# darglein/Snake-SLAM

Measured on AMD Instinct MI355X. Metric: frames/s ORB extract+match @752x480, higher is better.
Workload: dtype u8

## Files before the change

### snake_slam_amd/csrc/dispatch.hpp

```cpp
#pragma once
#include <cstddef>

#ifndef SNK_POSE_RED_STEPS
#define SNK_POSE_RED_STEPS 2
#endif

namespace snk
{
constexpr int BF_MFMA_MIN      = 24;
constexpr int BF_WIDE_MIN_WORK = 16384;

enum class Knn2Form { vector1, vector4, mfma };

inline Knn2Form knn2_form(int nq_cap, int nt_cap, int batch, bool no_mfma)
{
    if (!no_mfma && nq_cap >= BF_MFMA_MIN && nt_cap >= BF_MFMA_MIN) return Knn2Form::mfma;
    return (long long)batch * nq_cap >= BF_WIDE_MIN_WORK ? Knn2Form::vector4 : Knn2Form::vector1;
}

constexpr int BF_MFMA_WIDE_MIN_WGS = 512;

constexpr bool knn2_mfma_wide(int nq_cap, int , int batch, int wide_env)
{
    return wide_env >= 0 ? wide_env != 0 : (long long)batch * ((nq_cap + 255) / 256) >= BF_MFMA_WIDE_MIN_WGS;
}

constexpr int BF_MFMA_SHORT_NT = 8192;

constexpr bool knn2_mfma_short(int nt_cap, bool allowed) { return allowed && nt_cap <= BF_MFMA_SHORT_NT; }

constexpr int ST_SORT_MAX     = 8192;
constexpr int ST_FRAME_MAX    = 2560;
constexpr int ST_FRAME_BATCH  = 8;
constexpr int ST_COUNT_ROWS   = 4096;

enum class StereoForm { frame, count16, sort16, unindexed };

inline StereoForm stereo_host_form(int nr, bool sort_network)
{
    if (nr > ST_SORT_MAX) return StereoForm::unindexed;
    return sort_network ? StereoForm::sort16 : StereoForm::count16;
}

inline StereoForm stereo_batch_form(int nr_cap, int batch, bool no_frame_kernel, bool sort_network)
{
    if (!no_frame_kernel && nr_cap <= ST_FRAME_MAX && batch >= ST_FRAME_BATCH) return StereoForm::frame;
    return stereo_host_form(nr_cap, sort_network);
}

constexpr int POSE_SLOTS_PER_WAVE   = 64 >> SNK_POSE_RED_STEPS;
constexpr int POSE_HOST_WAVE4_MEAN  = 192;
constexpr int POSE_BATCH_WAVE4_MIN  = 256;
constexpr int POSE_TWO_PER_CU_BATCH = 256;
constexpr int POSE_MATCH_BYTES      = 56;

enum class PoseForm { wave1, wave2_lds, wave4_lds, wave4_global };

constexpr int pose_dyn_max() { return 160 * 1024 - (4 * POSE_SLOTS_PER_WAVE * 28 + 28) * 8 - 2048; }
constexpr int pose_two_per_cu() { return (80 * 1024 - (4 * POSE_SLOTS_PER_WAVE * 28 + 28) * 8 - 256) / POSE_MATCH_BYTES; }
constexpr int pose_four_per_cu() { return (160 * 1024 / 4 - (2 * POSE_SLOTS_PER_WAVE * 28 + 28) * 8 - 512) / POSE_MATCH_BYTES; }

inline PoseForm pose_host_form(size_t total, int n_problems, bool no_lds)
{
    if (total < (size_t)n_problems * POSE_HOST_WAVE4_MEAN) return PoseForm::wave1;
    return no_lds ? PoseForm::wave4_global : PoseForm::wave4_lds;
}

inline int pose_host_carve(int n_max, int n_problems)
{
    int lds_matches = n_max;
    if (n_problems > POSE_TWO_PER_CU_BATCH && lds_matches > pose_two_per_cu()) lds_matches = pose_two_per_cu();
    if ((size_t)lds_matches * POSE_MATCH_BYTES > (size_t)pose_dyn_max()) lds_matches = pose_dyn_max() / POSE_MATCH_BYTES;
    return lds_matches;
}

inline bool pose_batch_two_waves(int batch, int n_cu, int waves_env) { return waves_env == 2 || (waves_env != 4 && batch > 2 * n_cu); }

inline PoseForm pose_batch_form(int stride, int batch, int n_cu, int waves_env, bool no_lds)
{
    if (stride < POSE_BATCH_WAVE4_MIN) return PoseForm::wave1;
    if (no_lds) return PoseForm::wave4_global;
    return pose_batch_two_waves(batch, n_cu, waves_env) ? PoseForm::wave2_lds : PoseForm::wave4_lds;
}

inline int pose_batch_carve(int stride, int batch, int lds_env, bool two_waves)
{
    int lds_matches = stride;
    if (two_waves)
    {
        const int lm = lds_env > 0 ? lds_env : pose_four_per_cu();
        lds_matches  = lm < stride ? lm : stride;
    }
    else if (lds_env > 0) lds_matches = lds_env < stride ? lds_env : stride;
    else if (batch > POSE_TWO_PER_CU_BATCH && lds_matches > pose_two_per_cu()) lds_matches = pose_two_per_cu();
    if ((size_t)lds_matches * POSE_MATCH_BYTES > (size_t)pose_dyn_max()) lds_matches = pose_dyn_max() / POSE_MATCH_BYTES;
    return lds_matches;
}
}
```

### snake_slam_amd/csrc/matcher.hip

```cpp
#include "common.hpp"
#include "dispatch.hpp"

namespace snk
{
namespace
{
using u32 = unsigned int;
using u64 = unsigned long long;

constexpr u32 BF_IDX_BITS = 20;
constexpr u32 BF_IDX_MASK = (1u << BF_IDX_BITS) - 1u;
constexpr u32 BF_INF_KEY  = ((u32)SNK_DIST_INF << BF_IDX_BITS) | BF_IDX_MASK;

__device__ __forceinline__ int hamming256(const uint4& a0, const uint4& a1, const uint4& b0, const uint4& b1)
{
    return __popc(a0.x ^ b0.x) + __popc(a0.y ^ b0.y) + __popc(a0.z ^ b0.z) + __popc(a0.w ^ b0.w) +
           __popc(a1.x ^ b1.x) + __popc(a1.y ^ b1.y) + __popc(a1.z ^ b1.z) + __popc(a1.w ^ b1.w);
}

template <typename K>
__device__ __forceinline__ void merge2(K& k1, K& k2, K o1, K o2)
{
    K lo = k1 < o1 ? k1 : o1;
    K hi = k1 < o1 ? o1 : k1;
    K m  = k2 < o2 ? k2 : o2;
    k2   = hi < m ? hi : m;
    k1   = lo;
}

template <typename K>
__device__ __forceinline__ void insert2(K& k1, K& k2, K key)
{
    K hi = k1 < key ? key : k1;
    k1   = k1 < key ? k1 : key;
    k2   = k2 < hi ? k2 : hi;
}

template <int QW>
__global__ __launch_bounds__(256) void bf_knn2_kernel(const uint4* __restrict__ query, const int* __restrict__ nq_dev,
                                                      int nq_cap, int nq_host, const uint4* __restrict__ train,
                                                      const int* __restrict__ nt_dev, int nt_cap, int nt_host,
                                                      snk_knn2* __restrict__ out)
{
    const int b    = blockIdx.y;
    int nq         = nq_dev ? nq_dev[b] : nq_host;
    int nt         = nt_dev ? nt_dev[b] : nt_host;
    nq             = nq < nq_cap ? nq : nq_cap;
    nt             = nt < nt_cap ? nt : nt_cap;
    const int wave = __builtin_amdgcn_readfirstlane(threadIdx.x >> 6);
    const int lane = threadIdx.x & 63;
    const int q0   = (blockIdx.x * 4 + wave) * QW;
    if (q0 >= nq) return;

    const uint4* qb = query + (size_t)b * nq_cap * 2;
    const uint4* tb = train + (size_t)b * nt_cap * 2;

    uint4 qa[QW], qc[QW];
    u32 k1[QW], k2[QW];
#pragma unroll
    for (int k = 0; k < QW; ++k)
    {
        int qi = q0 + k < nq ? q0 + k : nq - 1;
        qa[k]  = qb[(size_t)qi * 2];
        qc[k]  = qb[(size_t)qi * 2 + 1];
        k1[k]  = BF_INF_KEY;
        k2[k]  = BF_INF_KEY;
    }

    for (int j = lane; j < nt; j += 64)
    {
        const uint4 ta = tb[(size_t)j * 2];
        const uint4 tc = tb[(size_t)j * 2 + 1];
#pragma unroll
        for (int k = 0; k < QW; ++k)
        {
            u32 d   = (u32)hamming256(qa[k], qc[k], ta, tc);
            u32 key = d < (u32)SNK_DIST_INF ? ((d << BF_IDX_BITS) | (u32)j) : BF_INF_KEY;
            insert2(k1[k], k2[k], key);
        }
    }

#pragma unroll
    for (int off = 32; off >= 1; off >>= 1)
    {
#pragma unroll
        for (int k = 0; k < QW; ++k)
        {
            u32 o1 = __shfl_xor(k1[k], off);
            u32 o2 = __shfl_xor(k2[k], off);
            merge2(k1[k], k2[k], o1, o2);
        }
    }

    if (lane == 0)
    {
#pragma unroll
        for (int k = 0; k < QW; ++k)
        {
            if (q0 + k < nq)
            {
                snk_knn2 r;
                r.dist1 = (int)(k1[k] >> BF_IDX_BITS);
                r.idx1  = (k1[k] & BF_IDX_MASK) == BF_IDX_MASK ? -1 : (int)(k1[k] & BF_IDX_MASK);
                r.dist2 = (int)(k2[k] >> BF_IDX_BITS);
                r.idx2  = (k2[k] & BF_IDX_MASK) == BF_IDX_MASK ? -1 : (int)(k2[k] & BF_IDX_MASK);
                out[(size_t)b * nq_cap + q0 + k] = r;
            }
        }
    }
}

typedef int v4i __attribute__((ext_vector_type(4)));
typedef int v16i __attribute__((ext_vector_type(16)));
constexpr int BFM_SENTINEL = 0x7F000000;
constexpr u32 BFS_IDX_BITS = 13;
static_assert(BF_MFMA_SHORT_NT == 1 << BFS_IDX_BITS, "the SHORT key's index field holds every index below BF_MFMA_SHORT_NT");

template <bool SHORT>
__device__ __forceinline__ v4i expand_bits(const uint4& h, int kc)
{
    if constexpr (SHORT)
    {
        const u32 M = 0x80808080u;
        return v4i{(int)((h.x << (7 - kc)) & M), (int)((h.y << (7 - kc)) & M), (int)((h.z << (7 - kc)) & M), (int)((h.w << (7 - kc)) & M)};
    }
    const u32 M = 0x01010101u;
    return v4i{(int)((h.x >> kc) & M), (int)((h.y >> kc) & M), (int)((h.z >> kc) & M), (int)((h.w >> kc) & M)};
}
__device__ __forceinline__ int popc128(const uint4& h) { return __popc(h.x) + __popc(h.y) + __popc(h.z) + __popc(h.w); }
__device__ __forceinline__ int med3s(int a, int b, int c) { return max(min(a, b), min(max(a, b), c)); }
template <bool MAXK>
__device__ __forceinline__ void insert2s(int& k1, int& k2, int key)
{
    k2 = med3s(k1, k2, key);
    k1 = MAXK ? max(k1, key) : min(k1, key);
}

template <int NB, bool SHORT>
__global__ __launch_bounds__(256, 2) void bf_knn2_mfma_kernel(const uint4* __restrict__ query, const int* __restrict__ nq_dev,
                                                              int nq_cap, int nq_host, const uint4* __restrict__ train,
                                                              const int* __restrict__ nt_dev, int nt_cap, int nt_host,
                                                              snk_knn2* __restrict__ out)
{
    __shared__ v4i As[2][8 * 2 * 32];
    __shared__ v16i ptk[2][2];
    constexpr int NONE = SHORT ? -BFM_SENTINEL : BFM_SENTINEL;
    const int b = blockIdx.y;
    int nq      = nq_dev ? nq_dev[b] : nq_host;
    int nt      = nt_dev ? nt_dev[b] : nt_host;
    nq          = nq < nq_cap ? nq : nq_cap;
    nt          = nt < nt_cap ? nt : nt_cap;
    if ((int)blockIdx.x * (128 * NB) >= nq) return;
    const int wave = __builtin_amdgcn_readfirstlane(threadIdx.x >> 6), lane = threadIdx.x & 63;
    const int j = lane & 31, g = lane >> 5;
    const int q0 = (blockIdx.x * 4 + wave) * (32 * NB);
    const uint4* qb = query + (size_t)b * nq_cap * 2;
    const uint4* tb = train + (size_t)b * nt_cap * 2;

    int pq[NB];
    v4i B[NB][8];
#pragma unroll
    for (int n = 0; n < NB; ++n)
    {
        const int qi   = min(q0 + 32 * n + j, nq - 1);
        const uint4 qh = qb[(size_t)qi * 2 + g], qo = qb[(size_t)qi * 2 + (1 - g)];
        pq[n]          = popc128(qh) + popc128(qo);
#pragma unroll
        for (int kc = 0; kc < 8; ++kc) {
            const v4i e = expand_bits<SHORT>(qh, kc);
            if constexpr (SHORT) B[n][kc] = e;
            else B[n][kc] = v4i{(int)((u32)e.x * 0xFFu), (int)((u32)e.y * 0xFFu), (int)((u32)e.z * 0xFFu), (int)((u32)e.w * 0xFFu)};
        }
    }

    const int e_i = wave * 8 + (lane & 7), e_g = (lane >> 3) & 1, e_k = lane >> 4;
    const int e_p = ((e_i >> 2) & 1) * 16 + (e_i & 3) + 4 * (e_i >> 3);
    const int ntiles = (nt + 31) >> 5;
    auto fetch = [&](int t, uint4& h)
    {
        const int ti = t * 32 + e_i;
        h = uint4{0u, 0u, 0u, 0u};
        if (ti < nt) h = tb[(size_t)ti * 2 + e_g];
    };
    auto expand = [&](int t, int buf, const uint4& h)
    {
        As[buf][((2 * e_k) * 2 + e_g) * 32 + e_i]     = expand_bits<SHORT>(h, 2 * e_k);
        As[buf][((2 * e_k + 1) * 2 + e_g) * 32 + e_i] = expand_bits<SHORT>(h, 2 * e_k + 1);
        const int ph = popc128(h);
        const int pt = ph + __shfl_down(ph, 8);
        if (lane < 8)
        {
            const int ti = t * 32 + e_i;
            const int k  = SHORT ? -((pt << BFS_IDX_BITS) | ti) : ((pt << BF_IDX_BITS) | ti);
            reinterpret_cast<int*>(&ptk[buf][0])[e_p] = ti < nt ? k : NONE;
        }
    };

    int k1[NB], k2[NB];
#pragma unroll
    for (int n = 0; n < NB; ++n) k1[n] = k2[n] = NONE;
    uint4 h;
    if (ntiles > 0)
    {
        fetch(0, h);
        expand(0, 0, h);
        if (ntiles > 1) fetch(1, h);
    }
    __syncthreads();
    for (int t = 0; t < ntiles; ++t)
    {
        const int buf = t & 1;
        if (t + 1 < ntiles)
        {
            expand(t + 1, buf ^ 1, h);
            if (t + 2 < ntiles) fetch(t + 2, h);
        }
        v16i acc[NB];
        v4i a[8];
#pragma unroll
        for (int kc = 0; kc < 8; ++kc) a[kc] = As[buf][(kc * 2 + g) * 32 + j];
        const v16i pk = ptk[buf][g];
#pragma unroll
        for (int n = 0; n < NB; ++n)
        {
            acc[n] = SHORT ? pk : v16i{0, 0, 0, 0, 0, 0, 0, 0, 0, 0, 0, 0, 0, 0, 0, 0};
#pragma unroll
            for (int kc = 0; kc < 8; ++kc) acc[n] = __builtin_amdgcn_mfma_i32_32x32x32_i8(a[kc], B[n][kc], acc[n], 0, 0, 0);
        }
#pragma unroll
        for (int n = 0; n < NB; ++n)
#pragma unroll
            for (int r = 0; r < 16; ++r)
            {
                if constexpr (SHORT) insert2s<true>(k1[n], k2[n], acc[n][r]);
                else insert2s<false>(k1[n], k2[n], (int)(((u32)acc[n][r] << (BF_IDX_BITS + 1)) + (u32)pk[r]));
            }
        __builtin_amdgcn_sched_group_barrier(0x100, SHORT ? 12 : 8, 0);
        __builtin_amdgcn_sched_group_barrier(0x008, 8, 0);
        if constexpr (!SHORT) __builtin_amdgcn_sched_group_barrier(0x100, 4, 0);
        __syncthreads();
    }
#pragma unroll
    for (int n = 0; n < NB; ++n)
    {
        const int o1 = __shfl_xor(k1[n], 32), o2 = __shfl_xor(k2[n], 32);
        int r1, r2;
        if constexpr (SHORT) r1 = -max(k1[n], o1), r2 = -max(min(k1[n], o1), max(k2[n], o2));
        else r1 = min(k1[n], o1), r2 = min(max(k1[n], o1), min(k2[n], o2));
        if (lane < 32 && q0 + 32 * n + lane < nq)
        {
            constexpr u32 IB = SHORT ? BFS_IDX_BITS : BF_IDX_BITS, IM = (1u << IB) - 1u;
            snk_knn2 r;
            const int a1 = r1 >= BFM_SENTINEL - (1 << 30) ? -1 : r1 + (pq[n] << IB);
            const int a2 = r2 >= BFM_SENTINEL - (1 << 30) ? -1 : r2 + (pq[n] << IB);
            const bool v1 = a1 >= 0 && (a1 >> IB) < SNK_DIST_INF, v2 = a2 >= 0 && (a2 >> IB) < SNK_DIST_INF;
            r.dist1 = v1 ? a1 >> IB : SNK_DIST_INF;
            r.idx1  = v1 ? (int)((u32)a1 & IM) : -1;
            r.dist2 = v2 ? a2 >> IB : SNK_DIST_INF;
            r.idx2  = v2 ? (int)((u32)a2 & IM) : -1;
            out[(size_t)b * nq_cap + q0 + 32 * n + lane] = r;
        }
    }
}

__global__ __launch_bounds__(256) void bf_filter_kernel(const snk_knn2* __restrict__ knn, const int* __restrict__ nq_dev,
                                                        int nq_cap, int nq_host, int threshold, float ratio, int th_strict,
                                                        int ratio_strict, int2* __restrict__ pairs, int* __restrict__ n_pairs)
{
    __shared__ int wave_cnt[4];
    __shared__ int base_s;
    const int b    = blockIdx.x;
    int nq         = nq_dev ? nq_dev[b] : nq_host;
    nq             = nq < nq_cap ? nq : nq_cap;
    const int tid  = threadIdx.x;
    const int wave = tid >> 6;
    const int lane = tid & 63;
    if (tid == 0) base_s = 0;
    __syncthreads();
    for (int start = 0; start < nq; start += 256)
    {
        const int i = start + tid;
        bool keep   = false;
        snk_knn2 k  = {};
        if (i < nq)
        {
            k    = knn[(size_t)b * nq_cap + i];
            const float rd2 = ratio * (float)k.dist2;
            keep = k.idx1 >= 0 && (th_strict ? k.dist1 < threshold : k.dist1 <= threshold) &&
                   (ratio_strict ? (float)k.dist1 < rd2 : (float)k.dist1 <= rd2);
        }
        const u64 mask   = __ballot(keep);
        const int prefix = __popcll(mask & ((1ull << lane) - 1ull));
        if (lane == 0) wave_cnt[wave] = __popcll(mask);
        __syncthreads();
        int off = base_s;
        for (int w = 0; w < wave; ++w) off += wave_cnt[w];
        if (keep) pairs[(size_t)b * nq_cap + off + prefix] = make_int2(i, k.idx1);
        __syncthreads();
        if (tid == 0) base_s += wave_cnt[0] + wave_cnt[1] + wave_cnt[2] + wave_cnt[3];
        __syncthreads();
    }
    if (tid == 0) n_pairs[b] = base_s;
}

struct LevelScales
{
    float s[32];
    int n;
    int iround_mode;
};

__device__ __forceinline__ int iround_d(double x, int mode)
{
    if (mode == 0) return (int)floor(x + 0.5);
    if (mode == 1) return (int)(x < 0.0 ? -floor(0.5 - x) : floor(x + 0.5));
    return (int)rint(x);
}

constexpr u64 ST_INF_KEY = (250ull << 40) | 0xFFFFFFFFFFull;
constexpr int ST_ROW_BIAS    = 4096;

__device__ __forceinline__ void stereo_sort_network(const snk_kp64* __restrict__ rb, int nr, int iround_mode, u32* keys, u32* __restrict__ out)
{
    const int tid = threadIdx.x;
    int n_pow2    = 2;
    while (n_pow2 < nr) n_pow2 <<= 1;
    for (int i = tid; i < n_pow2; i += 256)
    {
        u32 k = 0xFFFFFFFFu;
        if (i < nr)
        {
            int row = iround_d(rb[i].y, iround_mode) + ST_ROW_BIAS;
            row     = row < 0 ? 0 : (row > 65535 ? 65535 : row);
            k       = ((u32)row << 16) | (u32)i;
        }
        keys[i] = k;
    }
    __syncthreads();
    for (int k = 2; k <= n_pow2; k <<= 1)
        for (int j = k >> 1; j > 0; j >>= 1)
        {
            for (int t = tid; t < (n_pow2 >> 1); t += 256)
            {
                const int i   = ((t & ~(j - 1)) << 1) | (t & (j - 1));
                const int ixj = i | j;
                const bool up = (i & k) == 0;
                const u32 x = keys[i], y = keys[ixj];
                if ((x > y) == up)
                {
                    keys[i]   = y;
                    keys[ixj] = x;
                }
            }
            __syncthreads();
        }
    for (int i = tid; i < nr; i += 256) out[i] = keys[i];
}
__global__ __launch_bounds__(256) void stereo_sort_kernel(const snk_kp64* __restrict__ right, const int* __restrict__ nr_dev,
                                                          int nr_cap, int nr_host, int iround_mode, u32* __restrict__ row_sorted)
{
    extern __shared__ __attribute__((aligned(16))) unsigned char ssm[];
    const int b = blockIdx.x;
    int nr      = nr_dev ? nr_dev[b] : nr_host;
    nr          = nr < nr_cap ? nr : nr_cap;
    stereo_sort_network(right + (size_t)b * nr_cap, nr, iround_mode, reinterpret_cast<u32*>(ssm), row_sorted + (size_t)b * nr_cap);
}

__global__ __launch_bounds__(256) void stereo_count_kernel(const snk_kp64* __restrict__ right, const int* __restrict__ nr_dev, int nr_cap,
                                                           int nr_host, int iround_mode, u32* __restrict__ row_sorted,
                                                           int* __restrict__ n_matches, float* __restrict__ prefill_rp,
                                                           float* __restrict__ prefill_dp, int prefill_n)
{
    extern __shared__ __attribute__((aligned(16))) unsigned char ssm[];
    if (n_matches && threadIdx.x == 0) n_matches[blockIdx.x] = 0;
    if (prefill_rp)
        for (int i = threadIdx.x; i < prefill_n; i += 256)
        {
            prefill_rp[(size_t)blockIdx.x * prefill_n + i] = -1000.0f;
            prefill_dp[(size_t)blockIdx.x * prefill_n + i] = -1000.0f;
        }
    __shared__ int s_min, s_max, s_wsum[4];
    int* start   = reinterpret_cast<int*>(ssm);
    int* fill    = start + ST_COUNT_ROWS + 1;
    int* rowof   = fill + ST_COUNT_ROWS + 1;
    int* seg     = rowof + nr_cap;
    const int b = blockIdx.x, tid = threadIdx.x, lane = tid & 63, wave = tid >> 6;
    int nr      = nr_dev ? nr_dev[b] : nr_host;
    nr          = nr < nr_cap ? nr : nr_cap;
    const snk_kp64* rb = right + (size_t)b * nr_cap;
    if (tid == 0) s_min = 65535, s_max = 0;
    __syncthreads();
    int lmin = 65535, lmax = 0;
    for (int i = tid; i < nr; i += 256)
    {
        int row = iround_d(rb[i].y, iround_mode) + ST_ROW_BIAS;
        row     = row < 0 ? 0 : (row > 65535 ? 65535 : row);
        rowof[i] = row;
        lmin = min(lmin, row), lmax = max(lmax, row);
    }
    atomicMin(&s_min, lmin);
    atomicMax(&s_max, lmax);
    __syncthreads();
    const int r0 = s_min, span = nr > 0 ? s_max - s_min + 1 : 1;
    if (span > ST_COUNT_ROWS)
// ... 323 lines not shown
            row[u]  = min(row[u] - row0, ST_ROWS - 1);
            rank[u] = atomicAdd(&start[row[u]], 1);
        }
    __syncthreads();
    {
        const int a = start[2 * tid], c = start[2 * tid + 1];
        int x       = a + c;
        x = wave_scan_incl_dpp(x);
        if ((tid & 63) == 63) s_wtot[tid >> 6] = x;
        __syncthreads();
        int base = 0;
        for (int w = 0; w < (tid >> 6); ++w) base += s_wtot[w];
        const int excl     = base + x - (a + c);
        start[2 * tid]     = excl;
        start[2 * tid + 1] = excl + a;
        if (tid == 1023) start[ST_ROWS] = base + x;
    }
    __syncthreads();
#pragma unroll
    for (int u = 0; u < PER; ++u)
        if (row[u] >= 0) srt[start[row[u]] + rank[u]] = tid + 1024 * u;
    __syncthreads();

    constexpr int NGRP = 1024 / ST_GROUP;
    const int lane = tid % ST_GROUP, grp = tid / ST_GROUP;
    const float max_disp = (float)(bf * 0.5);
    snk_kp64 kp_n = lb[min(grp, nl - 1)];
    uint4 qa_n = dlb[(size_t)min(grp, nl - 1) * 2], qc_n = dlb[(size_t)min(grp, nl - 1) * 2 + 1];
    for (int i = grp; i < nl; i += NGRP)
    {
        const snk_kp64 kp = kp_n;
        const uint4 qa = qa_n, qc = qc_n;
        {
            const int in = min(i + NGRP, nl - 1);
            kp_n = lb[in];
            qa_n = dlb[(size_t)in * 2];
            qc_n = dlb[(size_t)in * 2 + 1];
        }
        const int y = iround_d(kp.y, ls.iround_mode);
        int oct     = kp.octave;
        oct         = oct < 0 ? 0 : (oct >= ls.n ? ls.n - 1 : oct);
        const int ri = (int)ceilf(2.0f * ls.s[oct]);
        const int lo_row  = min(max(y - ri + ST_ROW_BIAS, 0), 65535), hi_row = min(max(y + ri + ST_ROW_BIAS, 0), 65535);
        const int scan_lo = start[min(max(lo_row - row0, 0), ST_ROWS - 1)], scan_hi = start[min(max(hi_row - row0, 0), ST_ROWS - 1) + 1];
        u64 k1 = ST_INF_KEY, k2 = ST_INF_KEY;
        for (int pos = scan_lo + lane; pos < scan_hi; pos += ST_GROUP)
        {
            const int j   = srt[pos];
            const int rel = syj[j] - (y - ri);
            if (rel < 0 || rel > 2 * ri) continue;
            const double disparity = kp.x - sx[j];
            if (disparity < 0.0 || disparity > (double)max_disp) continue;
            int doct = kp.octave - soct[j];
            doct     = doct < 0 ? -doct : doct;
            if (doct > 1) continue;
            const int dist = hamming256(qa, qc, sdesc[2 * j], sdesc[2 * j + 1]);
            if (dist >= 250) continue;
            insert2(k1, k2, ((u64)dist << 40) | ((u64)rel << 24) | (u64)j);
        }
#pragma unroll
        for (int off = ST_GROUP / 2; off >= 1; off >>= 1)
        {
            const u64 o1 = __shfl_xor(k1, off, 16), o2 = __shfl_xor(k2, off, 16);
            merge2(k1, k2, o1, o2);
        }
        if (lane != 0) continue;
        const int best_dist = (int)(k1 >> 40), second_best_dist = (int)(k2 >> 40);
        if (best_dist > (relaxed ? 75 : 40)) continue;
        if ((double)best_dist > (relaxed ? 0.9 : 0.7) * (double)second_best_dist) continue;
        const int best_id  = (int)(k1 & 0xFFFFFFull);
        const float angle1 = kp.angle, angle2 = sang[best_id];
        const float rot    = fminf(fabsf(angle1 - angle2), fminf(fabsf((angle1 + 365.0f) - angle2), fabsf(angle1 - (angle2 + 365.0f))));
        if (rot > (relaxed ? 25.0f : 5.0f)) continue;
        double right_point = sx[best_id];
        double disparity   = kp.x - right_point;
        if (disparity <= 0.001)
        {
            disparity   = 0.001;
            right_point = kp.x - disparity;
        }
        right_points[(size_t)b * nl_cap + i] = (float)right_point;
        depth[(size_t)b * nl_cap + i]        = (float)(bf / disparity);
        atomicAdd(&s_cnt, 1);
    }
    __syncthreads();
    if (tid == 0) n_matches[b] = s_cnt;
}
}
}

using namespace snk;

#include "matcher_handle.hpp"

extern "C" {

int snk_matcher_destroy(snk_matcher* m);

int snk_matcher_create(int device, void* stream, snk_matcher** out)
{
    SNK_REQUIRE(out != nullptr, "out is NULL");
    *out           = nullptr;
    snk_matcher* m = new snk_matcher();
    int rc         = m->init(device, stream);
    constexpr size_t SCRATCH = 4u << 20;
    for (snk::DevBuf* b : {&m->q, &m->t, &m->out, &m->aux, &m->aux2, &m->view})
        if (rc == SNK_OK) rc = b->reserve(SCRATCH);
    if (rc == SNK_OK) rc = m->cnt.reserve(256);
    if (rc == SNK_OK) rc = m->h_in.reserve(1u << 20);
    if (rc == SNK_OK) rc = m->h_res.reserve(256u << 10);
    if (rc != SNK_OK)
    {
        snk_matcher_destroy(m);
        return rc;
    }
    *out = m;
    return SNK_OK;
}

int snk_matcher_destroy(snk_matcher* m)
{
    if (!m) return SNK_OK;
    (void)hipSetDevice(m->device);
    m->q.release();
    m->t.release();
    m->out.release();
    m->aux.release();
    m->aux2.release();
    m->cnt.release();
    m->view.release();
    m->h_in.release();
    m->h_res.release();
    m->sim3_its.release();
    m->sim3_its_host.release();
    m->fini();
    delete m;
    return SNK_OK;
}

int snk_matcher_sync(snk_matcher* m)
{
    SNK_REQUIRE(m != nullptr, "matcher is NULL");
    SNK_HIP_CHECK(hipStreamSynchronize(m->stream));
    return SNK_OK;
}

static int launch_knn2(snk_matcher* m, const uint64_t* q, const int32_t* nq_dev, int nq_cap, int nq_host,
                       const uint64_t* t, const int32_t* nt_dev, int nt_cap, int nt_host, int batch, snk_knn2* out)
{
    if (batch <= 0 || nq_cap <= 0) return SNK_OK;
    static const bool no_mfma = getenv("SNK_BF_NO_MFMA") != nullptr;
    static const int wide_env  = getenv("SNK_BF_MFMA_WIDE") ? (atoi(getenv("SNK_BF_MFMA_WIDE")) != 0 ? 1 : 0) : -1;
    static const bool short_env = getenv("SNK_BF_MFMA_NO_SHORT") == nullptr;
    switch (knn2_form(nq_cap, nt_cap, batch, no_mfma))
    {
    case Knn2Form::mfma:
    {
        const bool wide = knn2_mfma_wide(nq_cap, nt_cap, batch, wide_env), shrt = knn2_mfma_short(nt_cap, short_env);
        auto kernel = wide ? (shrt ? bf_knn2_mfma_kernel<2, true> : bf_knn2_mfma_kernel<2, false>)
                           : (shrt ? bf_knn2_mfma_kernel<1, true> : bf_knn2_mfma_kernel<1, false>);
        hipLaunchKernelGGL(kernel, dim3(ceil_div(nq_cap, wide ? 256 : 128), batch), dim3(256), 0, m->stream, (const uint4*)q, nq_dev, nq_cap,
                           nq_host, (const uint4*)t, nt_dev, nt_cap, nt_host, out);
    }
        break;
    case Knn2Form::vector4:
        hipLaunchKernelGGL(bf_knn2_kernel<4>, dim3(ceil_div(nq_cap, 16), batch), dim3(256), 0, m->stream, (const uint4*)q, nq_dev, nq_cap,
                           nq_host, (const uint4*)t, nt_dev, nt_cap, nt_host, out);
        break;
    case Knn2Form::vector1:
        hipLaunchKernelGGL(bf_knn2_kernel<1>, dim3(ceil_div(nq_cap, 4), batch), dim3(256), 0, m->stream, (const uint4*)q, nq_dev, nq_cap,
                           nq_host, (const uint4*)t, nt_dev, nt_cap, nt_host, out);
        break;
    }
    SNK_LAUNCH_CHECK();
    return SNK_OK;
}

int snk_bf_knn2(snk_matcher* m, const uint64_t (*query)[4], int nq, const uint64_t (*train)[4], int nt, snk_knn2* out)
{
    SNK_REQUIRE(m != nullptr, "matcher is NULL");
    SNK_REQUIRE(nq >= 0 && nt >= 0, "negative count");
    SNK_REQUIRE(nt < (int)BF_IDX_MASK, "train set too large (max 2^20-2)");
    if (nq == 0) return SNK_OK;
    SNK_REQUIRE(query != nullptr && out != nullptr, "NULL buffer");
    SNK_REQUIRE(nt == 0 || train != nullptr, "NULL train buffer");
    SNK_HIP_CHECK(hipSetDevice(m->device));
    int rc;
    const size_t qb = (size_t)nq * 32, tb = (size_t)(nt > 0 ? nt : 1) * 32, ob = (size_t)nq * sizeof(snk_knn2);
    if ((rc = m->q.reserve(qb + tb)) != SNK_OK) return rc;
    if ((rc = m->out.reserve(ob)) != SNK_OK) return rc;
    if ((rc = m->h_in.reserve(qb + tb)) != SNK_OK) return rc;
    if ((rc = m->h_res.reserve(ob)) != SNK_OK) return rc;
    memcpy(m->h_in.p, query, qb);
    if (nt > 0) memcpy(m->h_in.as<char>() + qb, train, (size_t)nt * 32);
    SNK_HIP_CHECK(hipMemcpyAsync(m->q.p, m->h_in.p, qb + (nt > 0 ? (size_t)nt * 32 : 0), hipMemcpyHostToDevice, m->stream));
    rc = launch_knn2(m, m->q.as<uint64_t>(), nullptr, nq, nq, reinterpret_cast<const uint64_t*>(m->q.as<char>() + qb), nullptr,
                     nt > 0 ? nt : 1, nt, 1, m->out.as<snk_knn2>());
    if (rc != SNK_OK) return rc;
    SNK_HIP_CHECK(hipMemcpyAsync(m->h_res.p, m->out.p, ob, hipMemcpyDeviceToHost, m->stream));
    SNK_HIP_CHECK(hipStreamSynchronize(m->stream));
    memcpy(out, m->h_res.p, ob);
    return SNK_OK;
}

int snk_bf_knn2_batch_dev(snk_matcher* m, const uint64_t* query_dev, const int32_t* nq_dev, int nq_cap,
                          const uint64_t* train_dev, const int32_t* nt_dev, int nt_cap, int batch, snk_knn2* out_dev)
{
    SNK_REQUIRE(m != nullptr, "matcher is NULL");
    SNK_REQUIRE(batch >= 0 && nq_cap >= 0 && nt_cap >= 1, "bad sizes");
    SNK_REQUIRE(nt_cap < (int)BF_IDX_MASK, "train capacity too large (max 2^20-2)");
    SNK_REQUIRE(query_dev && train_dev && out_dev && nq_dev && nt_dev, "NULL device buffer");
    SNK_HIP_CHECK(hipSetDevice(m->device));
    return launch_knn2(m, query_dev, nq_dev, nq_cap, 0, train_dev, nt_dev, nt_cap, 0, batch, out_dev);
}

int snk_bf_filter(snk_matcher* m, const snk_knn2* knn, int nq, int threshold, float ratio, int32_t (*pairs)[2],
                  int* n_pairs)
{
    SNK_REQUIRE(m != nullptr, "matcher is NULL");
    SNK_REQUIRE(nq >= 0, "negative count");
    SNK_REQUIRE(n_pairs != nullptr, "n_pairs is NULL");
    *n_pairs = 0;
    if (nq == 0) return SNK_OK;
    SNK_REQUIRE(knn != nullptr && pairs != nullptr, "NULL buffer");
    SNK_HIP_CHECK(hipSetDevice(m->device));
    int rc;
    const size_t kb = (size_t)nq * sizeof(snk_knn2), pb = 16 + (size_t)nq * 8;
    if ((rc = m->out.reserve(kb)) != SNK_OK) return rc;
    if ((rc = m->aux.reserve(pb)) != SNK_OK) return rc;
    if ((rc = m->h_in.reserve(kb)) != SNK_OK) return rc;
    if ((rc = m->h_res.reserve(pb)) != SNK_OK) return rc;
    memcpy(m->h_in.p, knn, kb);
    SNK_HIP_CHECK(hipMemcpyAsync(m->out.p, m->h_in.p, kb, hipMemcpyHostToDevice, m->stream));
    hipLaunchKernelGGL(bf_filter_kernel, dim3(1), dim3(256), 0, m->stream, m->out.as<snk_knn2>(), (const int*)nullptr,
                       nq, nq, threshold, ratio, definition(DEF_BF_FILTER_THRESHOLD_STRICT), definition(DEF_BF_FILTER_RATIO_STRICT),
                       reinterpret_cast<int2*>(m->aux.as<char>() + 16), m->aux.as<int>());
    SNK_LAUNCH_CHECK();
    SNK_HIP_CHECK(hipMemcpyAsync(m->h_res.p, m->aux.p, pb, hipMemcpyDeviceToHost, m->stream));
    SNK_HIP_CHECK(hipStreamSynchronize(m->stream));
    const int n = *m->h_res.as<int>();
    if (n > 0) memcpy(pairs, m->h_res.as<char>() + 16, (size_t)n * 8);
    *n_pairs = n;
    return SNK_OK;
}

int snk_bf_filter_batch_dev(snk_matcher* m, const snk_knn2* knn_dev, const int32_t* nq_dev, int nq_cap, int batch,
                            int threshold, float ratio, int32_t* pairs_dev, int32_t* n_pairs_dev)
{
    SNK_REQUIRE(m != nullptr, "matcher is NULL");
    SNK_REQUIRE(batch >= 0 && nq_cap >= 0, "bad sizes");
    SNK_REQUIRE(knn_dev && nq_dev && pairs_dev && n_pairs_dev, "NULL device buffer");
    if (batch == 0) return SNK_OK;
    SNK_HIP_CHECK(hipSetDevice(m->device));
    hipLaunchKernelGGL(bf_filter_kernel, dim3(batch), dim3(256), 0, m->stream, knn_dev, nq_dev, nq_cap, 0, threshold,
                       ratio, definition(DEF_BF_FILTER_THRESHOLD_STRICT), definition(DEF_BF_FILTER_RATIO_STRICT), (int2*)pairs_dev,
                       n_pairs_dev);
    SNK_LAUNCH_CHECK();
    return SNK_OK;
}

static int make_scales(const float* level_scale, int n_levels, LevelScales* ls)
{
    SNK_REQUIRE(level_scale != nullptr && n_levels >= 1 && n_levels <= 32, "level_scale / n_levels (1..32)");
    for (int i = 0; i < 32; ++i) ls->s[i] = i < n_levels ? level_scale[i] : level_scale[n_levels - 1];
    ls->n           = n_levels;
    ls->iround_mode = definition(DEF_IROUND_MODE);
    return SNK_OK;
}

int snk_stereo_match(snk_matcher* m, const snk_kp64* left, const uint64_t (*desc_left)[4], int nl,
                     const snk_kp64* right, const uint64_t (*desc_right)[4], int nr, double bf, const float* level_scale,
                     int n_levels, int relaxed, float* right_points, float* depth, int* n_matches)
{
    SNK_REQUIRE(m != nullptr, "matcher is NULL");
    SNK_REQUIRE(nl >= 0 && nr >= 0, "negative count");
    SNK_REQUIRE(n_matches != nullptr, "n_matches is NULL");
    SNK_REQUIRE(nr < (1 << 24), "right set too large");
    *n_matches = 0;
    LevelScales ls;
    int rc = make_scales(level_scale, n_levels, &ls);
    if (rc != SNK_OK) return rc;
    if (nl == 0 || nr == 0) return SNK_OK;
    SNK_REQUIRE(left && desc_left && right && desc_right && right_points && depth, "NULL buffer");
    SNK_HIP_CHECK(hipSetDevice(m->device));
    const size_t kl = (size_t)nl * sizeof(snk_kp64), kr = (size_t)nr * sizeof(snk_kp64);
    auto al16 = [](size_t v) { return (v + 15) & ~(size_t)15; };
    const size_t o_kr = al16(kl), o_dl = al16(o_kr + kr), o_dr = al16(o_dl + (size_t)nl * 32), o_rp = al16(o_dr + (size_t)nr * 32);
    const size_t o_dp = o_rp + (size_t)nl * 4, o_cnt = o_dp + (size_t)nl * 4, in_b = o_cnt + 4, res_b = in_b - o_rp;
    if ((rc = m->aux.reserve(in_b)) != SNK_OK) return rc;
    if ((rc = m->h_in.reserve(in_b)) != SNK_OK) return rc;
    if ((rc = m->h_res.reserve(res_b)) != SNK_OK) return rc;
    char* ab   = m->aux.as<char>();
    char* hb   = m->h_in.as<char>();
    float* rp  = reinterpret_cast<float*>(ab + o_rp);
    float* dp  = reinterpret_cast<float*>(ab + o_dp);
    int* d_cnt = reinterpret_cast<int*>(ab + o_cnt);
    const uint4* d_dl = reinterpret_cast<const uint4*>(ab + o_dl);
    const uint4* d_dr = reinterpret_cast<const uint4*>(ab + o_dr);
    memcpy(hb, left, kl);
    memcpy(hb + o_kr, right, kr);
    memcpy(hb + o_dl, desc_left, (size_t)nl * 32);
    memcpy(hb + o_dr, desc_right, (size_t)nr * 32);
    memcpy(hb + o_rp, right_points, (size_t)nl * 4);
    memcpy(hb + o_dp, depth, (size_t)nl * 4);
    memset(hb + o_cnt, 0, 4);
    SNK_HIP_CHECK(hipMemcpyAsync(ab, hb, in_b, hipMemcpyHostToDevice, m->stream));
    const u32* srt = nullptr;
    static const bool sort_network = getenv("SNK_STEREO_SORT_NETWORK") != nullptr;
    const StereoForm form = stereo_host_form(nr, sort_network);
    if (form != StereoForm::unindexed)
    {
        if ((rc = m->out.reserve((size_t)nr * 4)) != SNK_OK) return rc;
        int np2 = 2;
// ... 114 lines not shown
```

Baseline: 199,100.

## Add FP4 scaled-MFMA brute-force kNN2 kernel for short train sets

Adds a new brute-force Hamming kNN2 kernel that expands each descriptor bit into an FP4 nibble and computes dot products with the MI355X scaled f8f6f4 32x32x64 MFMA. Top-2 tracking is done in float keys with fmed3. The kernel is selected by default whenever the short-key MFMA path applies (nt_cap <= 8192), and can be disabled with an environment variable. The aim is higher matrix throughput per instruction than the existing integer MFMA path. In exchange it adds bit-expansion work and float key-packing precision constraints.

```diff
diff --git a/snake_slam_amd/csrc/dispatch.hpp b/snake_slam_amd/csrc/dispatch.hpp
--- a/snake_slam_amd/csrc/dispatch.hpp
+++ b/snake_slam_amd/csrc/dispatch.hpp
@@ -28,6 +28,8 @@
 constexpr int BF_MFMA_SHORT_NT = 8192;
 
 constexpr bool knn2_mfma_short(int nt_cap, bool allowed) { return allowed && nt_cap <= BF_MFMA_SHORT_NT; }
+
+constexpr bool knn2_mfma_fp4(int nt_cap, bool short_keys, bool allowed) { return allowed && short_keys && nt_cap <= BF_MFMA_SHORT_NT; }
 
 constexpr int ST_SORT_MAX     = 8192;
 constexpr int ST_FRAME_MAX    = 2560;
diff --git a/snake_slam_amd/csrc/knn2_fp4.hpp b/snake_slam_amd/csrc/knn2_fp4.hpp
--- /dev/null
+++ b/snake_slam_amd/csrc/knn2_fp4.hpp
@@ -0,0 +1,26 @@
+#pragma once
+
+namespace snk
+{
+namespace fp4
+{
+typedef int v4i __attribute__((ext_vector_type(4)));
+typedef int v8i __attribute__((ext_vector_type(8)));
+typedef float v16f __attribute__((ext_vector_type(16)));
+
+constexpr int SCALE_2_7 = (int)0x86868686u;
+
+__device__ __forceinline__ v4i expand_fp4(const uint4& h, int s)
+{
+    const unsigned m = 0x11111111u << s, r = (unsigned)(s + 31) & 31u;
+    return v4i{(int)__builtin_rotateright32(h.x & m, r), (int)__builtin_rotateright32(h.y & m, r), (int)__builtin_rotateright32(h.z & m, r),
+               (int)__builtin_rotateright32(h.w & m, r)};
+}
+
+__device__ __forceinline__ v16f mfma_fp4(const v4i& a, const v4i& b, const v16f& acc)
+{
+    const v8i a8 = __builtin_shufflevector(a, a, 0, 1, 2, 3, -1, -1, -1, -1), b8 = __builtin_shufflevector(b, b, 0, 1, 2, 3, -1, -1, -1, -1);
+    return __builtin_amdgcn_mfma_scale_f32_32x32x64_f8f6f4(a8, b8, acc, 4, 4, 0, SCALE_2_7, 0, SCALE_2_7);
+}
+}
+}
diff --git a/snake_slam_amd/csrc/matcher.hip b/snake_slam_amd/csrc/matcher.hip
--- a/snake_slam_amd/csrc/matcher.hip
+++ b/snake_slam_amd/csrc/matcher.hip
@@ -1,5 +1,6 @@
 #include "common.hpp"
 #include "dispatch.hpp"
+#include "knn2_fp4.hpp"
 
 namespace snk
 {
@@ -250,6 +251,128 @@
         if (lane < 32 && q0 + 32 * n + lane < nq)
         {
             constexpr u32 IB = SHORT ? BFS_IDX_BITS : BF_IDX_BITS, IM = (1u << IB) - 1u;
+            snk_knn2 r;
+            const int a1 = r1 >= BFM_SENTINEL - (1 << 30) ? -1 : r1 + (pq[n] << IB);
+            const int a2 = r2 >= BFM_SENTINEL - (1 << 30) ? -1 : r2 + (pq[n] << IB);
+            const bool v1 = a1 >= 0 && (a1 >> IB) < SNK_DIST_INF, v2 = a2 >= 0 && (a2 >> IB) < SNK_DIST_INF;
+            r.dist1 = v1 ? a1 >> IB : SNK_DIST_INF;
+            r.idx1  = v1 ? (int)((u32)a1 & IM) : -1;
+            r.dist2 = v2 ? a2 >> IB : SNK_DIST_INF;
+            r.idx2  = v2 ? (int)((u32)a2 & IM) : -1;
+            out[(size_t)b * nq_cap + q0 + 32 * n + lane] = r;
+        }
+    }
+}
+
+constexpr float BFK_ABOVE = 8388608.0f;
+__device__ __forceinline__ void insert2f(float& k1, float& k2, float key)
+{
+    k2 = __builtin_amdgcn_fmed3f(k1, k2, key);
+    k1 = __builtin_amdgcn_fmed3f(k1, key, BFK_ABOVE);
+}
+
+template <int NB>
+__global__ __launch_bounds__(256, 2) void bf_knn2_mfma_fp4_kernel(const uint4* __restrict__ query, const int* __restrict__ nq_dev,
+                                                                  int nq_cap, int nq_host, const uint4* __restrict__ train,
+                                                                  const int* __restrict__ nt_dev, int nt_cap, int nt_host,
+                                                                  snk_knn2* __restrict__ out)
+{
+    using fp4::v16f;
+    __shared__ v4i As[2][4 * 2 * 32];
+    __shared__ v16f ptk[2][2];
+    constexpr float NONE = -(float)BFM_SENTINEL;
+    const int b = blockIdx.y;
+    int nq      = nq_dev ? nq_dev[b] : nq_host;
+    int nt      = nt_dev ? nt_dev[b] : nt_host;
+    nq          = nq < nq_cap ? nq : nq_cap;
+    nt          = nt < nt_cap ? nt : nt_cap;
+    if ((int)blockIdx.x * (128 * NB) >= nq) return;
+    const int wave = __builtin_amdgcn_readfirstlane(threadIdx.x >> 6), lane = threadIdx.x & 63;
+    const int j = lane & 31, g = lane >> 5;
+    const int q0 = (blockIdx.x * 4 + wave) * (32 * NB);
+    const uint4* qb = query + (size_t)b * nq_cap * 2;
+    const uint4* tb = train + (size_t)b * nt_cap * 2;
+
+    int pq[NB];
+    v4i B[NB][4];
+#pragma unroll
+    for (int n = 0; n < NB; ++n)
+    {
+        const int qi   = min(q0 + 32 * n + j, nq - 1);
+        const uint4 qh = qb[(size_t)qi * 2 + g], qo = qb[(size_t)qi * 2 + (1 - g)];
+        pq[n]          = popc128(qh) + popc128(qo);
+#pragma unroll
+        for (int s = 0; s < 4; ++s) B[n][s] = fp4::expand_fp4(qh, s);
+    }
+
+    const int e_i = wave * 8 + (lane & 7), e_g = (lane >> 3) & 1, e_s = lane >> 4;
+    const int e_p = ((e_i >> 2) & 1) * 16 + (e_i & 3) + 4 * (e_i >> 3);
+    const int ntiles = (nt + 31) >> 5;
+    auto fetch = [&](int t, uint4& h)
+    {
+        const int ti = t * 32 + e_i;
+        h = uint4{0u, 0u, 0u, 0u};
+        if (ti < nt) h = tb[(size_t)ti * 2 + e_g];
+    };
+    auto expand = [&](int t, int buf, const uint4& h)
+    {
+        As[buf][(e_s * 2 + e_g) * 32 + e_i] = fp4::expand_fp4(h, e_s);
+        const int ph = popc128(h);
+        const int pt = ph + __shfl_down(ph, 8);
+        if (lane < 8)
+        {
+            const int ti = t * 32 + e_i;
+            reinterpret_cast<float*>(&ptk[buf][0])[e_p] = ti < nt ? -(float)((pt << BFS_IDX_BITS) | ti) : NONE;
+        }
+    };
+
+    float k1[NB], k2[NB];
+#pragma unroll
+    for (int n = 0; n < NB; ++n) k1[n] = k2[n] = NONE;
+    uint4 h;
+    if (ntiles > 0)
+    {
+        fetch(0, h);
+        expand(0, 0, h);
+        if (ntiles > 1) fetch(1, h);
+    }
+    __syncthreads();
+    for (int t = 0; t < ntiles; ++t)
+    {
+        const int buf = t & 1;
+        if (t + 1 < ntiles)
+        {
+            expand(t + 1, buf ^ 1, h);
+            if (t + 2 < ntiles) fetch(t + 2, h);
+        }
+        v16f acc[NB];
+        v4i a[4];
+#pragma unroll
+        for (int s = 0; s < 4; ++s) a[s] = As[buf][(s * 2 + g) * 32 + j];
+        const v16f pk = ptk[buf][g];
+#pragma unroll
+        for (int n = 0; n < NB; ++n)
+        {
+            acc[n] = pk;
+#pragma unroll
+            for (int s = 0; s < 4; ++s) acc[n] = fp4::mfma_fp4(a[s], B[n][s], acc[n]);
+        }
+#pragma unroll
+        for (int n = 0; n < NB; ++n)
+#pragma unroll
+            for (int r = 0; r < 16; ++r) insert2f(k1[n], k2[n], acc[n][r]);
+        __builtin_amdgcn_sched_group_barrier(0x100, 8, 0);
+        __builtin_amdgcn_sched_group_barrier(0x008, 4, 0);
+        __syncthreads();
+    }
+#pragma unroll
+    for (int n = 0; n < NB; ++n)
+    {
+        const float o1 = __shfl_xor(k1[n], 32), o2 = __shfl_xor(k2[n], 32);
+        const int r1 = -(int)fmaxf(k1[n], o1), r2 = -(int)fmaxf(fminf(k1[n], o1), fmaxf(k2[n], o2));
+        if (lane < 32 && q0 + 32 * n + lane < nq)
+        {
+            constexpr u32 IB = BFS_IDX_BITS, IM = (1u << IB) - 1u;
             snk_knn2 r;
             const int a1 = r1 >= BFM_SENTINEL - (1 << 30) ? -1 : r1 + (pq[n] << IB);
             const int a2 = r2 >= BFM_SENTINEL - (1 << 30) ? -1 : r2 + (pq[n] << IB);
@@ -879,6 +1002,7 @@
     static const bool no_mfma = getenv("SNK_BF_NO_MFMA") != nullptr;
     static const int wide_env  = getenv("SNK_BF_MFMA_WIDE") ? (atoi(getenv("SNK_BF_MFMA_WIDE")) != 0 ? 1 : 0) : -1;
     static const bool short_env = getenv("SNK_BF_MFMA_NO_SHORT") == nullptr;
+    static const bool fp4_env   = getenv("SNK_BF_MFMA_NO_FP4") == nullptr;
     switch (knn2_form(nq_cap, nt_cap, batch, no_mfma))
     {
     case Knn2Form::mfma:
@@ -886,6 +1010,7 @@
         const bool wide = knn2_mfma_wide(nq_cap, nt_cap, batch, wide_env), shrt = knn2_mfma_short(nt_cap, short_env);
         auto kernel = wide ? (shrt ? bf_knn2_mfma_kernel<2, true> : bf_knn2_mfma_kernel<2, false>)
                            : (shrt ? bf_knn2_mfma_kernel<1, true> : bf_knn2_mfma_kernel<1, false>);
+        if (knn2_mfma_fp4(nt_cap, shrt, fp4_env)) kernel = wide ? bf_knn2_mfma_fp4_kernel<2> : bf_knn2_mfma_fp4_kernel<1>;
         hipLaunchKernelGGL(kernel, dim3(ceil_div(nq_cap, wide ? 256 : 128), batch), dim3(256), 0, m->stream, (const uint4*)q, nq_dev, nq_cap,
                            nq_host, (const uint4*)t, nt_dev, nt_cap, nt_host, out);
     }
```

Result: no change. 201,000, median of 6 (+0.9%).
